# jamesmshihua/DiffusionPolicyOptimization

Measured on AMD Instinct MI355X. Metric: env-steps/sec + PPO-updates/sec, hopper-v2 64 envs 20 DDPM steps, 1/2/4/8 GPU, higher is better.
Workload: dtype bf16; 1 GPU; hopper-medium-v2 DPPO fine-tune iteration: 64 envs/GPU x 500 chunks (Ta=4), K=20 DDPM steps (K'=10), 5 PPO epochs x minibatch 50000, bf16 denoiser, synthetic linear env; env=synthetic, global_envs=64, chunks_per_rollout=500, parallelism=single GPU, batch_semantics=global minibatch 50000 rows = the reference's (50000 per rank)

## Files before the change

### diffusionpolicyoptimization_amd/csrc/update.hip

```cpp
#include <stdlib.h>
#include <mutex>
#include <vector>
#include "dppo_ppo.h"

enum { EXTRA_NONE = 0, EXTRA_ONES = 1, EXTRA_ONEHOT = 2 };
#define DW_MAXP 8
#define DW_TN 128
#ifndef DPPO_DW_LINE
#define DPPO_DW_LINE 128
#endif
#define DW_LINE DPPO_DW_LINE
#define DW_CPL (DW_LINE / 16)
#define DW_FPI (64 / DW_CPL)
#define DW_BOPB (DW_TN * DW_LINE)
static_assert(DW_LINE == 64 || DW_LINE == 128, "DPPO_DW_LINE must be 64 or 128");

template <int WK, int RC = 8> struct DWGeom {
    static constexpr int W = WK / 32;
    static constexpr int AOPB = WK * DW_LINE;
    static constexpr int SLOT = AOPB + DW_BOPB + 1024;
    static constexpr int RING0 = 160 * 1024 / SLOT < 8 ? 160 * 1024 / SLOT : 8;
    static constexpr int RING = RING0 < RC ? RING0 : RC;
    static constexpr int AI = WK / DW_FPI / W;
    static constexpr int BI = DW_TN / DW_FPI / W;
    static_assert(RING * SLOT <= 160 * 1024, "dW ring exceeds the CU's LDS");
};

struct DWProb {
    const void* XT; const void* DT; float* G; float* Gx;
    int Kx, N, extra, ktiles, ntiles;
};
struct DWArgs {
    DWProb p[DW_MAXP];
    int tile_start[DW_MAXP + 1];
    int nprob, nchunks, mchunk;
    float out_scale;
    size_t ldm;
    const int8_t* seg;
    const int* rows_dev;
};

typedef __attribute__((address_space(3))) void lds_void_t;

template <class P>
__device__ inline u32x4 extra_frag(int extra, int q, const int8_t* seg_lds) {
    using AT = typename P::AT;
    AT e[P::EPL];
    if (extra == EXTRA_ONES) {
#pragma unroll
        for (int i = 0; i < P::EPL; ++i) e[i] = P::cvt(1.f);
    } else {
        const uint64_t w = P::EPL == 8 ? *reinterpret_cast<const uint64_t*>(seg_lds)
                                       : (uint64_t)*reinterpret_cast<const uint32_t*>(seg_lds);
#pragma unroll
        for (int i = 0; i < P::EPL; ++i) e[i] = P::cvt((int)(int8_t)(w >> (8 * i)) == q ? 1.f : 0.f);
    }
    return __builtin_bit_cast(u32x4, e);
}

__device__ inline int dw_swz(int f, int c) {
    if constexpr (DW_LINE == 128) return c ^ (f & 7);
    else return c ^ ((0x78 >> (2 * ((f >> 2) & 3))) & 3);
}
__device__ inline u32x4 dw_lds_frag(const uint8_t* img, int f, int c) {
    return *reinterpret_cast<const u32x4*>(img + f * DW_LINE + (dw_swz(f, c) << 4));
}

template <int N>
__device__ inline void vm_wait() {
    static_assert(N >= 0 && N < 64, "vmcnt is 6 bits");
    __builtin_amdgcn_s_waitcnt((N & 15) | ((N >> 4) << 14) | (7 << 4) | (15 << 8));
}

template <class P, int WK, int RC, bool EXTRA, bool SEGLD>
__device__ __forceinline__ void dw_loop(uint8_t* smem, const DWArgs& a, const DWProb& pr, int nst, size_t m_begin,
                                        int wave, int lane, const typename P::AT* const (&srcA)[DWGeom<WK, RC>::AI],
                                        const typename P::AT* const (&srcB)[DWGeom<WK, RC>::BI],
                                        f32x4 (&acc)[4][4], f32x4 (&acce)[4]) {
    using G = DWGeom<WK, RC>;
    constexpr int BK = DW_LINE / (int)sizeof(typename P::AT);
    constexpr int OPS = G::AI + G::BI + (SEGLD ? 1 : 0);
    const int wr = wave >> 1, wc = wave & 1;
    const int fr = lane & 15, cq = lane >> 4;
    auto issue = [&](int st) {
        uint8_t* base = smem + (st % G::RING) * G::SLOT;
        const size_t off = (size_t)st * BK;
#pragma unroll
        for (int i = 0; i < G::AI; ++i)
            __builtin_amdgcn_global_load_lds((void*)(srcA[i] + off), (lds_void_t*)(base + (wave + G::W * i) * 1024), 16,
                                             0, 0);
#pragma unroll
        for (int i = 0; i < G::BI; ++i)
            __builtin_amdgcn_global_load_lds((void*)(srcB[i] + off),
                                             (lds_void_t*)(base + G::AOPB + (wave + G::W * i) * 1024), 16, 0, 0);
        if constexpr (SEGLD) {
            const int8_t* sg = a.seg + m_begin + off + 4 * (lane < BK / 4 ? lane : 0);
            __builtin_amdgcn_global_load_lds((void*)sg, (lds_void_t*)(base + G::AOPB + DW_BOPB), 4, 0, 0);
        }
    };
#pragma unroll
    for (int p = 0; p < G::RING - 1; ++p)
        if (p < nst) issue(p);
    for (int st = 0; st < nst; ++st) {
        const int ahead = nst - 1 - st;
        if (ahead >= G::RING - 2) vm_wait<(G::RING - 2) * OPS>();
        else if (ahead == 1) vm_wait<OPS>();
        else vm_wait<0>();
        __builtin_amdgcn_s_barrier();
        asm volatile("" ::: "memory");
        if (st + G::RING - 1 < nst) issue(st + G::RING - 1);
        const uint8_t* imA = smem + (st % G::RING) * G::SLOT;
        const uint8_t* imB = imA + G::AOPB;
        const int8_t* seg_lds = (const int8_t*)(imB + DW_BOPB);
#pragma unroll
        for (int ks = 0; ks < DW_LINE / 64; ++ks) {
            u32x4 A[4], B[4];
#pragma unroll
            for (int i = 0; i < 4; ++i) {
                A[i] = dw_lds_frag(imA, wr * 64 + i * 16 + fr, ks * 4 + cq);
                B[i] = dw_lds_frag(imB, wc * 64 + i * 16 + fr, ks * 4 + cq);
            }
#pragma unroll
            for (int i = 0; i < 4; ++i)
#pragma unroll
                for (int j = 0; j < 4; ++j) acc[i][j] = P::mma(A[i], B[j], acc[i][j]);
            if constexpr (EXTRA) {
                const u32x4 AE = extra_frag<P>(pr.extra, fr, seg_lds + ks * P::KG + cq * P::EPL);
#pragma unroll
                for (int j = 0; j < 4; ++j) acce[j] = P::mma(AE, B[j], acce[j]);
            }
        }
    }
}

static int dw_device_cus() {
    static int n = [] {
        int dev = 0, c = 0;
        if (hipGetDevice(&dev) != hipSuccess || hipDeviceGetAttribute(&c, hipDeviceAttributeMultiprocessorCount, dev) != hipSuccess)
            c = 256;
        return c > 0 ? c : 256;
    }();
    return n;
}

template <class P, int WK, int RC>
__global__ __launch_bounds__(WK / 32 * 64) void dw_kernel(DWArgs a) {
    using AT = typename P::AT;
    using G = DWGeom<WK, RC>;
    constexpr int BK = DW_LINE / (int)sizeof(AT);
    constexpr int EPC = 16 / (int)sizeof(AT);
    __shared__ __attribute__((aligned(1024))) uint8_t smem[G::RING * G::SLOT];
    const int tid = threadIdx.x, lane = tid & 63, wave = tid >> 6;
    const int tiles_all = a.tile_start[a.nprob];
    const int total = tiles_all * a.nchunks;
    const int per = (total + 7) >> 3;
    const int lg = (int)(blockIdx.x & 7) * per + (int)(blockIdx.x >> 3);
    if (lg >= total) return;
    const int chunk = lg / tiles_all;
    const int tile = lg % tiles_all;
    int pi = 0;
    while (pi + 1 < a.nprob && tile >= a.tile_start[pi + 1]) ++pi;
    const DWProb& pr = a.p[pi];
    const int lt = tile - a.tile_start[pi];
    const int kt = lt / pr.ntiles, nt = lt % pr.ntiles;
    const int k_base = kt * WK, n_base = nt * DW_TN;
    const int wr = wave >> 1, wc = wave & 1;
    size_t lim = a.ldm, mchunk = (size_t)a.mchunk;
    if (a.rows_dev) {
        const size_t d64 = (size_t)(__builtin_amdgcn_readfirstlane(*a.rows_dev) + 63) / 64 * 64;
        lim = d64 < lim ? d64 : lim;
        mchunk = (lim + (size_t)a.nchunks * 64 - 1) / ((size_t)a.nchunks * 64) * 64;
    }
    const size_t m_begin = (size_t)chunk * mchunk;
    const size_t m_end = m_begin + mchunk < lim ? m_begin + mchunk : lim;
    if (m_begin >= m_end) return;
    const int nst = (int)((m_end - m_begin) / BK);
    const AT* XT = (const AT*)pr.XT;
    const AT* DT = (const AT*)pr.DT;
    const bool wg_extra = pr.extra != EXTRA_NONE && kt == 0;
    const bool do_extra = wg_extra && wr == 0;
    const bool seg_ld = do_extra && pr.extra == EXTRA_ONEHOT;

    const AT* srcA[G::AI];
    const AT* srcB[G::BI];
#pragma unroll
    for (int i = 0; i < G::AI; ++i) {
        const int f = (wave + G::W * i) * DW_FPI + lane / DW_CPL;
        const int c = dw_swz(f, lane % DW_CPL);
        int fa = k_base + f; fa = fa < pr.Kx ? fa : pr.Kx - 1;
        srcA[i] = XT + (size_t)fa * a.ldm + m_begin + c * EPC;
    }
#pragma unroll
    for (int i = 0; i < G::BI; ++i) {
        const int f = (wave + G::W * i) * DW_FPI + lane / DW_CPL;
        const int c = dw_swz(f, lane % DW_CPL);
        int fb = n_base + f; fb = fb < pr.N ? fb : pr.N - 1;
        srcB[i] = DT + (size_t)fb * a.ldm + m_begin + c * EPC;
    }
    f32x4 acc[4][4], acce[4];
#pragma unroll
    for (int i = 0; i < 4; ++i) {
        zero_acc(acce[i]);
#pragma unroll
        for (int j = 0; j < 4; ++j) zero_acc(acc[i][j]);
    }
    if (seg_ld) dw_loop<P, WK, RC, true, true>(smem, a, pr, nst, m_begin, wave, lane, srcA, srcB, acc, acce);
    else if (do_extra) dw_loop<P, WK, RC, true, false>(smem, a, pr, nst, m_begin, wave, lane, srcA, srcB, acc, acce);
    else dw_loop<P, WK, RC, false, false>(smem, a, pr, nst, m_begin, wave, lane, srcA, srcB, acc, acce);
#pragma unroll
    for (int i = 0; i < 4; ++i)
#pragma unroll
        for (int j = 0; j < 4; ++j) {
            const int n = n_base + wc * 64 + j * 16 + ccol(lane);
#pragma unroll
            for (int r = 0; r < 4; ++r) {
                const int k = k_base + wr * 64 + i * 16 + crow(lane, r);
                if (k < pr.Kx && n < pr.N) atomicAdd(pr.G + (size_t)k * pr.N + n, acc[i][j][r] * a.out_scale);
            }
        }
    if (do_extra) {
#pragma unroll
        for (int j = 0; j < 4; ++j) {
            const int n = n_base + wc * 64 + j * 16 + ccol(lane);
            if (n >= pr.N) continue;
#pragma unroll
            for (int r = 0; r < 4; ++r) {
                const int q = crow(lane, r);
                if (pr.extra == EXTRA_ONES) {
                    if (q == 0) atomicAdd(pr.Gx + n, acce[j][r] * a.out_scale);
                } else {
                    atomicAdd(pr.Gx + (size_t)q * pr.N + n, acce[j][r] * a.out_scale);
                }
            }
        }
    }
}

#ifndef TB_THREADS
#define TB_THREADS 1024
#endif
struct L2Back {
    const float* pl2;
    const float* gob;
    const uint8_t* wimg;
    float* gw;
    float* gb;
    int H, N, prec;
    uint32_t* zcnt;
    const int* zlist;
    const int* zn;
};
__device__ inline float packed_elem(const uint8_t* img, int K, int k, int n, int prec) {
    const bool two = prec == DPPO_BF16 || prec == DPPO_F16;
    const int KG = two ? 32 : 16, EPL = two ? 8 : 4;
    const int lane = (n & 15) + 16 * ((k % KG) / EPL);
    const size_t slot = ((size_t)(n >> 4) * packed_ksteps(K, KG) + k / KG) * 64 + lane;
    const uint8_t* e = img + slot * 16 + (size_t)(k % EPL) * (two ? 2 : 4);
    if (prec == DPPO_BF16) return (float)*(const __bf16*)e;
    if (prec == DPPO_F16) return (float)*(const _Float16*)e;
    return *(const float*)e;
}
template <int PREC>
__device__ inline float packed_elem_t(const uint8_t* img, int K, int k, int n) {
    constexpr bool two = PREC == DPPO_BF16 || PREC == DPPO_F16;
    constexpr int KG = two ? 32 : 16, EPL = two ? 8 : 4;
    const int lane = (n & 15) + 16 * ((k % KG) / EPL);
    const size_t slot = ((size_t)(n >> 4) * packed_ksteps(K, KG) + k / KG) * 64 + lane;
    const uint8_t* e = img + slot * 16 + (size_t)(k % EPL) * (two ? 2 : 4);
    if constexpr (PREC == DPPO_BF16) return (float)*(const __bf16*)e;
    else if constexpr (PREC == DPPO_F16) return (float)*(const _Float16*)e;
    else return *(const float*)e;
}
constexpr int L2B_ROWS = 4;
constexpr int L2B_MAXN = 32;
template <int PREC, int NJ, int NQ>
__device__ inline void l2_back_cols(const L2Back& a, int b, int t, int nt) {
    const int H = a.H, N = NQ < L2B_MAXN ? NQ : a.N;
    const int h0 = L2B_ROWS * b;
    float pv[L2B_ROWS + 1][NQ];
#pragma unroll
    for (int r = 0; r < L2B_ROWS; ++r)
#pragma unroll
        for (int q = 0; q < NQ; ++q) pv[r][q] = q < N ? a.pl2[(size_t)(h0 + r) * N + q] : 0.f;
#pragma unroll
    for (int q = 0; q < NQ; ++q) pv[L2B_ROWS][q] = q < N ? a.gob[q] : 0.f;
    constexpr int NW = NQ <= 16 ? NJ : 1;
    float w[NW][NQ];
    auto load_w = [&](int c, float* dst) {
// ... 1064 lines not shown

extern "C" int dppo_feistel_permute(int64_t first, int64_t count, int64_t n, uint64_t seed, int epoch, int64_t* out,
                                    void* stream) {
    DPPO_CHECK(n > 0 && count >= 0 && first >= 0, "dppo_feistel_permute: bad range");
    if (count == 0) return DPPO_OK;
    DPPO_CHECK(out, "dppo_feistel_permute: null out");
    const FeistelKey fk = feistel_key((uint64_t)n, seed, epoch);
    hipLaunchKernelGGL(feistel_kernel, dim3((unsigned)((count + 255) / 256)), dim3(256), 0, (hipStream_t)stream,
                       first, count, fk, out);
    DPPO_HIP(hipGetLastError());
    return DPPO_OK;
}

extern "C" int dppo_ppo_adv_stats(const float* advantages, int64_t total, int K_ft, uint64_t perm_seed, int epoch,
                                  int64_t start, int rows, const int64_t* row_index, double* adv_stats, void* stream) {
    DPPO_CHECK(advantages && adv_stats && total > 0 && K_ft > 0 && rows >= 0, "dppo_ppo_adv_stats: bad args");
    hipStream_t s = (hipStream_t)stream;
    DPPO_HIP(hipMemsetAsync(adv_stats, 0, 3 * sizeof(double), s));
    if (rows == 0) return DPPO_OK;
    const FeistelKey fk = feistel_key((uint64_t)total, perm_seed, epoch);
    const int blocks = dppo_cdiv(rows, 256) < 512 ? dppo_cdiv(rows, 256) : 512;
    hipLaunchKernelGGL(adv_stats_kernel, dim3(blocks), dim3(256), 0, s, advantages, fk, K_ft, start, rows, row_index,
                       adv_stats);
    DPPO_HIP(hipGetLastError());
    return DPPO_OK;
}

extern "C" int dppo_ppo_adv_stats_all(const float* advantages, int64_t total, int K_ft, uint64_t perm_seed, int epoch0,
                                      int n_epochs, int64_t rows_full, int n_batch, double* adv_stats, void* stream) {
    DPPO_CHECK(advantages && adv_stats && total > 0 && K_ft > 0 && rows_full > 0 && n_batch > 0 && n_epochs > 0,
               "dppo_ppo_adv_stats_all: bad args");
    DPPO_CHECK(n_epochs <= ADV_MAXE, "dppo_ppo_adv_stats_all: at most %d epochs", ADV_MAXE);
    DPPO_CHECK((uint64_t)total < ((uint64_t)1 << 32), "dppo_ppo_adv_stats_all: total exceeds 2^32");
    hipStream_t s = (hipStream_t)stream;
    const int nm = n_epochs * n_batch;
    DPPO_HIP(hipMemsetAsync(adv_stats, 0, (size_t)3 * nm * sizeof(double), s));
    AdvStatsAll a = {};
    for (int e = 0; e < n_epochs; ++e) a.fk[e] = feistel_key((uint64_t)total, perm_seed, epoch0 + e);
    a.nbatch = n_batch; a.KF = K_ft; a.rows_full = rows_full; a.total = total;
    const int64_t bx = dppo_cdiv((int)(rows_full < total ? rows_full : total), 256);
    const int blocks = bx < 64 ? (int)bx : 64;
    DppoKtScope kt(KT_ADV_STATS, s);
    hipLaunchKernelGGL(adv_stats_all_kernel, dim3(blocks, nm), dim3(256), 0, s, advantages, a, adv_stats);
    DPPO_HIP(hipGetLastError());
    return DPPO_OK;
}

extern "C" size_t dppo_ppo_workspace_bytes(const dppo_dims* d, int precision, int batch_rows) {
    Dims D;
    if (dppo_check_dims(d, &D) || batch_rows < 0) return 0;
    return make_ppo_workspace(D, precision, batch_rows, nullptr).total;
}

template <class P>
static int launch_dw(const DWArgs& a, int wk, hipStream_t s) {
    const int tiles = a.tile_start[a.nprob];
    const int64_t blocks = 8 * (((int64_t)tiles * a.nchunks + 7) / 8);
    if (wk == 256)
        hipLaunchKernelGGL((dw_kernel<P, 256, 8>), dim3((unsigned)blocks), dim3(DWGeom<256>::W * 64), 0, s, a);
    else if (wk == 128)
        hipLaunchKernelGGL((dw_kernel<P, 128, 8>), dim3((unsigned)blocks), dim3(DWGeom<128>::W * 64), 0, s, a);
    else
        hipLaunchKernelGGL((dw_kernel<P, 128, 3>), dim3((unsigned)blocks), dim3(128 / 32 * 64), 0, s, a);
    DPPO_HIP(hipGetLastError());
    return DPPO_OK;
}

constexpr int DW_TK = 256;

struct SideStream { hipStream_t stream; hipEvent_t fork, join; };
static SideStream* side_stream() {
    constexpr int MAXDEV = 16;
    thread_local SideStream ss[MAXDEV] = {};
    thread_local bool tried[MAXDEV] = {};
    int dev = 0;
    if (hipGetDevice(&dev) != hipSuccess || dev < 0 || dev >= MAXDEV) return nullptr;
    SideStream& e = ss[dev];
    if (!tried[dev]) {
        tried[dev] = true;
        if (hipStreamCreateWithFlags(&e.stream, hipStreamNonBlocking) != hipSuccess ||
            hipEventCreateWithFlags(&e.fork, hipEventDisableTiming) != hipSuccess ||
            hipEventCreateWithFlags(&e.join, hipEventDisableTiming) != hipSuccess) {
            (void)hipGetLastError();
            e.stream = nullptr;
        }
    }
    return e.stream ? &e : nullptr;
}


static int launch_time_bwd(const Dims& D, int precision, const float* gseg, const float* pl2, const float* pa0,
                           const void* packed_actor, const float* actor_params, float* ga, int nb, int TS, hipStream_t s,
                           bool l2_back = true) {
    const FlatOffsets FA = make_flat_offsets(D.IN, D.H, D.XD, D.TD);
    const MlpLayout L = make_mlp_layout(D.IN, D.H, D.XD, D.TD, precision, D.K);
    L2Back l2b = {pl2, ga + FA.out_b, (const uint8_t*)packed_actor + L.off[SEG_W_OUT], ga + FA.l2_w, ga + FA.l2_b, D.H,
                  D.XD, precision, nullptr, nullptr, nullptr};
    DPPO_CHECK(D.XD <= L2B_MAXN, "l2_back: action horizon x dim %d > %d", D.XD, L2B_MAXN);
    DPPO_CHECK(D.IN <= 256 && D.H % 4 == 0, "out_back: in_dim %d > 256", D.IN);
    int stage_g = 0;
    const size_t tsm0 = time_bwd_lds(D, nb, &stage_g);
    const size_t tsm = tsm0 > sizeof(float) * OB_RED * (TB_THREADS / 256) ? tsm0 : sizeof(float) * OB_RED * (TB_THREADS / 256);
    DPPO_CHECK(tsm <= 160 * 1024, "time_bwd: LDS staging %zu B exceeds 160 KB", tsm);
    const int per = TB_THREADS / 256;
    const int l2g = l2_back ? dppo_cdiv(D.H, L2B_ROWS) : 0, obg = dppo_cdiv(D.H, ob_rows(l2_nq(D.XD)));
    const int nq = l2_nq(D.XD);
    const void* fn = time_l2_bwd_fn(precision, nq);
    { const int rc_ = dppo_func_lds(fn, tsm); if (rc_) return rc_; }
    DppoKtScope kt(KT_TIME_BWD, s);
    const OutBack ob = make_out_back(D, precision, actor_params, pl2, pa0, ga);
    const dim3 grid(1 + dppo_cdiv(l2g > obg ? l2g : obg, per));
    int XD = D.XD, TD = D.TD, H = D.H;
    FlatOffsets fa = FA;
    const float* prm = actor_params;
    void* args[] = {(void*)&gseg, (void*)&prm, (void*)&ga, (void*)&fa, (void*)&XD, (void*)&TD, (void*)&H, (void*)&nb,
                    (void*)&TS, (void*)&stage_g, (void*)&l2b, (void*)&l2g, (void*)&ob, (void*)&obg};
    DPPO_HIP(hipLaunchKernel(fn, grid, dim3(TB_THREADS), args, tsm, s));
    DPPO_HIP(hipGetLastError());
    return DPPO_OK;
}

// ... 70 lines not shown
    const PpoWorkspace ws = make_ppo_workspace(D, precision, rows, (uint8_t*)workspace);
    DPPO_CHECK(ws.total < ((size_t)1 << 31), "dppo_ppo_minibatch: workspace for %d rows exceeds 2 GiB", rows);
    const FlatOffsets FA = make_flat_offsets(D.IN, D.H, D.XD, D.TD);
    const FlatOffsets FC = make_flat_offsets(D.SD, D.HC, 1, 0);
    float* ga = grads;
    float* gc = grads + FA.count;
    DPPO_CHECK(parts >= 1 && parts <= 5, "dppo_ppo_minibatch: bad part %d", parts);
    DPPO_CHECK(parts == 3 || adv_stats || parts == 2 || parts == 5,
               "dppo_ppo_minibatch_part: the actor half needs adv_stats");
    DPPO_CHECK((hp->flags & ~(DPPO_PPO_L2_DEFERRED | DPPO_PPO_LEARN_ETA | DPPO_PPO_PRECLEARED)) == 0,
               "dppo_ppo_minibatch: unknown flags 0x%x", hp->flags);
    const ZeroArgs z = minibatch_zero_args(D, ws, grads, metrics, parts);
    if (parts != 5 && !(hp->flags & DPPO_PPO_PRECLEARED)) {
        DppoKtScope kt(KT_ZERO, s);
        hipLaunchKernelGGL(zero_kernel, dim3(16), dim3(256), 0, s, z);
        DPPO_HIP(hipGetLastError());
    }
    DPPO_CHECK((uint64_t)total < ((uint64_t)1 << 32), "dppo_ppo_minibatch: %lld samples x steps exceed 2^32",
               (long long)total);
    const FeistelKey fk = feistel_key((uint64_t)total, perm_seed, epoch);
    const double* stats = adv_stats;
    if (!stats && parts != 2 && parts != 5) {
        const int blocks = dppo_cdiv(rows, 256) < 512 ? dppo_cdiv(rows, 256) : 512;
        hipLaunchKernelGGL(adv_stats_kernel, dim3(blocks), dim3(256), 0, s, advantages, fk, D.KF, start, rows,
                           row_index, ws.stats);
        DPPO_HIP(hipGetLastError());
        stats = ws.stats;
    }
    LossHP lh;
    lh.gamma_denoising = hp->gamma_denoising; lh.clip_coef = hp->clip_ploss_coef;
    lh.clip_coef_base = hp->clip_ploss_coef_base; lh.clip_coef_rate = hp->clip_ploss_coef_rate;
    lh.min_lp_std = hp->min_logprob_std; lh.vf_coef = hp->vf_coef; lh.norm_adv = hp->norm_adv;
    lh.reward_horizon = hp->reward_horizon;
    const float gscale = dppo_grad_scale_rows(precision, hp->global_rows);
    lh.grad_scale = hp->loss_scale / (float)hp->global_rows * gscale;
    lh.eta_unscale = (hp->flags & DPPO_PPO_LEARN_ETA) ? 1.f / gscale : 0.f;
    lh.clip_vloss = hp->clip_vloss_coef > 0.f && hp->old_values ? hp->clip_vloss_coef : 0.f;
    lh.old_values = lh.clip_vloss > 0.f ? hp->old_values : nullptr;
    const bool l2_def = (hp->flags & DPPO_PPO_L2_DEFERRED) != 0;

    ActorArgs aa = {};
    aa.packed = (const uint8_t*)packed_ft;
    aa.L = make_mlp_layout(D.IN, D.H, D.XD, D.TD, precision, D.K);
    aa.sched = sched; aa.obs = obs; aa.chains = chains;
    aa.XD = D.XD; aa.SD = D.SD; aa.TD = D.TD; aa.IN = D.IN; aa.H = D.H; aa.KF = D.KF; aa.Da = D.Da; aa.TS = D.TS;
    aa.mode = ROWS_TRAIN; aa.nrows = rows; aa.fk = fk; aa.start = start; aa.row_index = row_index;
    aa.lp_old = lp_old_mean; aa.adv = advantages; aa.adv_stats = stats; aa.hp = lh; aa.ws = ws; aa.metrics = metrics;

    CriticArgs ca = {};
    ca.packed = (const uint8_t*)packed_critic;
    ca.L = make_mlp_layout(D.SD, D.HC, 1, 0, precision);
    ca.obs = obs; ca.SD = D.SD; ca.HC = D.HC; ca.KF = D.KF; ca.mode = ROWS_TRAIN; ca.nrows = rows;
    ca.fk = fk; ca.start = start; ca.row_index = row_index; ca.returns = returns; ca.hp = lh; ca.ws = ws; ca.metrics = metrics;
    const int tk = DW_TK;
    const int* crit_rows_dev = nullptr;
    auto launch_grads = [&](bool actor, hipStream_t st) -> int {
        DWArgs w = {};
        int all_tiles = 0;
        if (!actor) w.rows_dev = crit_rows_dev;
        const size_t span = ws.ldm;
        const int wk = actor ? tk : 0, tke = wk ? wk : 128;
        auto add = [&](const void* XT, int Kx, const void* DT, int N, float* G, int extra, float* Gx) {
            all_tiles += dppo_cdiv(Kx, tke) * dppo_cdiv(N, DW_TN);
            DWProb& p = w.p[w.nprob];
            p.XT = XT; p.DT = DT; p.G = G; p.Gx = Gx; p.Kx = Kx; p.N = N; p.extra = extra;
            p.ktiles = dppo_cdiv(Kx, tke); p.ntiles = dppo_cdiv(N, DW_TN);
            w.tile_start[w.nprob + 1] = w.tile_start[w.nprob] + p.ktiles * p.ntiles;
            w.nprob++;
        };
        if (actor) {
            add(ws.a0T, D.IN, ws.dh1T, D.H, ga + FA.in_w, EXTRA_ONEHOT, ws.gseg);
            add(ws.u1T, D.H, ws.dh2T, D.H, ga + FA.l1_w, EXTRA_ONES, ga + FA.l1_b);
            add(ws.u2T, D.H, ws.dyT, D.XD, l2_def ? ga + FA.l2_w : ws.pl2, EXTRA_NONE, nullptr);
            add(ws.a0T, D.IN, ws.dyT, D.XD, ws.pa0, EXTRA_ONES, ga + FA.out_b);
        } else {
            add(ws.csT, D.SD, ws.cdh1T, D.HC, gc + FC.in_w, EXTRA_ONES, gc + FC.in_b);
            add(ws.cu1T, D.HC, ws.cdh2T, D.HC, gc + FC.l1_w, EXTRA_ONES, gc + FC.l1_b);
            add(ws.cu2T, D.HC, ws.cdvT, 1, ws.cpl2, EXTRA_NONE, nullptr);
            add(ws.ch3T, D.HC, ws.cdvT, 1, gc + FC.out_w, EXTRA_ONES, gc + FC.out_b);
        }
        w.ldm = ws.ldm;
        w.seg = ws.seg;
        w.out_scale = 1.f / gscale;
        const int tiles = all_tiles;
        int nch = dw_device_cus() / tiles;
        if (nch > (int)(span / 768)) nch = (int)(span / 768);
        const int max_ch = (int)(span / 64);
        if (nch > max_ch) nch = max_ch;
        if (nch < 1) nch = 1;
        w.mchunk = (int)(dppo_cdiv((int)span, nch * 64) * 64);
        w.nchunks = dppo_cdiv((int)span, w.mchunk);
        DppoKtScope kt(actor ? KT_DW_ACTOR : KT_DW_CRITIC, st);
        return precision == DPPO_BF16 ? launch_dw<PolicyBF16>(w, wk, st)
             : precision == DPPO_F16  ? launch_dw<PolicyF16>(w, wk, st) : launch_dw<PolicyF32>(w, wk, st);
    };

    uint32_t* crit_cnt = nullptr;
    auto critic_rows = [&](hipStream_t st) -> int {
        if (!crit_dedup()) return DPPO_OK;
        const int64_t nsamp = total / D.KF;
        { const int rc_ = crit_count_scratch(nsamp, st, &crit_cnt); if (rc_) return rc_; }
        const int blocks = dppo_cdiv(rows, 256) < 512 ? dppo_cdiv(rows, 256) : 512;
        DppoKtScope kt(KT_CRIT_ROWS, st);
        hipLaunchKernelGGL(crit_rows_kernel, dim3(blocks), dim3(256), 0, st, row_index, start, rows, fk, D.KF, crit_cnt,
                           ws.crow_n, ws.crow_cnt);
        DPPO_HIP(hipGetLastError());
        ca.crow_n = ws.crow_n; ca.crow_mult = crit_cnt; ca.crow_cnt = ws.crow_cnt;
        crit_rows_dev = ws.crow_cnt;
        return DPPO_OK;
    };
    auto critic_tail = [&](hipStream_t st) {
        return launch_critic_l2_back(D, precision, ws.cpl2, packed_critic, gc, crit_cnt, ws.crow_n, ws.crow_cnt, st);
    };

    const float* pl2_src = l2_def ? ga + FA.l2_w : ws.pl2;
    auto actor_grads = [&]() -> int { return launch_grads(true, s); };
    auto actor_tail = [&]() -> int {
        return launch_time_bwd(D, precision, ws.gseg, pl2_src, ws.pa0, packed_ft, actor_params, ga, D.KF, D.TS, s,
                               !l2_def);
    };

    if (parts == 2) {
        rc = critic_rows(s);
        if (rc) return rc;
        rc = launch_critic_rowtile(ca, precision, s);
        if (rc) return rc;
        rc = launch_grads(false, s);
        if (rc) return rc;
        return critic_tail(s);
    }
    if (parts == 1 || parts == 4 || parts == 5) {
        if (parts != 5) {
            rc = launch_actor_rowtile(aa, precision, s);
            if (rc) return rc;
        }
        if (parts == 4) return DPPO_OK;
        rc = actor_grads();
        if (rc) return rc;
        return actor_tail();
    }
    SideStream* side = side_stream();
    if (side) {
        DPPO_HIP(hipEventRecord(side->fork, s));
        DPPO_HIP(hipStreamWaitEvent(side->stream, side->fork, 0));
        rc = critic_rows(side->stream);
        if (rc) return rc;
        rc = launch_critic_rowtile(ca, precision, side->stream);
// ... 76 lines not shown
__global__ __launch_bounds__(256) void seg_reduce_kernel(const AT* __restrict__ dT, const int8_t* __restrict__ seg,
                                                         size_t ldm, int nb, float* __restrict__ G, int H, float scale) {
    __shared__ float bins[4][64];
    const int n = blockIdx.x, tid = threadIdx.x, wave = tid >> 6;
    for (int i = tid; i < 4 * 64; i += 256) (&bins[0][0])[i] = 0.f;
    __syncthreads();
    const AT* row = dT + (size_t)n * ldm;
#pragma unroll 4
    for (size_t r = tid; r < ldm; r += 256) {
        const int q = seg[r];
        if (q >= 0 && q < nb) atomicAdd(&bins[wave][q], (float)row[r]);
    }
    __syncthreads();
    if (tid < nb) G[(size_t)tid * H + n] = ((bins[0][tid] + bins[1][tid]) + (bins[2][tid] + bins[3][tid])) * scale;
}

extern "C" int dppo_pretrain_minibatch(const dppo_dims* d, int precision, const void* packed_actor, const float* actor_params,
                                       const float* sched, const float* qsched, const float* x_start, const float* cond,
                                       const int32_t* t, const float* noise, int rows, int64_t global_rows,
                                       float loss_scale, void* workspace, float* grads, double* metrics, void* stream) {
    Dims D;
    int rc = dppo_check_dims(d, &D);
    if (rc) return rc;
    DPPO_CHECK(dppo_prec_ok(precision), "bad precision %d", precision);
    DPPO_CHECK(packed_actor && actor_params && sched && qsched && x_start && cond && t && noise && workspace && grads &&
               metrics, "dppo_pretrain_minibatch: null pointer");
    DPPO_CHECK(rows > 0 && global_rows >= rows, "dppo_pretrain_minibatch: bad rows / global_rows");
    DPPO_CHECK(D.TS == 1, "dppo_pretrain_minibatch: the time-embedding table must be unstrided (time_stride 1)");
    DPPO_CHECK(D.K <= 64, "dppo_pretrain_minibatch: denoising_steps > 64 unsupported (bucket sums)");
    hipStream_t s = (hipStream_t)stream;
    const PpoWorkspace ws = make_ppo_workspace(D, precision, rows, (uint8_t*)workspace);
    DPPO_CHECK(ws.total < ((size_t)1 << 31), "dppo_pretrain_minibatch: workspace for %d rows exceeds 2 GiB", rows);
    const FlatOffsets FA = make_flat_offsets(D.IN, D.H, D.XD, D.TD);
    float* ga = grads;
    ZeroArgs z = {};
    z.p[0] = grads; z.n[0] = FA.count * sizeof(float);
    z.p[1] = metrics; z.n[1] = 16 * sizeof(double);
    z.p[2] = ws.pl2; z.n[2] = (size_t)((const uint8_t*)ws.gseg - (const uint8_t*)ws.pl2);
    hipLaunchKernelGGL(zero_kernel, dim3(256), dim3(256), 0, s, z);
    DPPO_HIP(hipGetLastError());

    ActorArgs aa = {};
    aa.packed = (const uint8_t*)packed_actor;
    aa.L = make_mlp_layout(D.IN, D.H, D.XD, D.TD, precision, D.K);
    aa.sched = sched; aa.obs = cond; aa.chains = x_start;
    aa.XD = D.XD; aa.SD = D.SD; aa.TD = D.TD; aa.IN = D.IN; aa.H = D.H; aa.KF = D.K; aa.Da = D.Da; aa.TS = 1;
    aa.mode = ROWS_PRETRAIN; aa.nrows = rows; aa.ws = ws; aa.metrics = metrics;
    aa.tsteps = t; aa.noise = noise; aa.qsched = qsched;
    const float gscale = dppo_grad_scale_rows(precision, global_rows);
    aa.pre_scale = 2.f * loss_scale / ((float)global_rows * (float)D.XD) * gscale;
    rc = launch_actor_rowtile(aa, precision, s);
    if (rc) return rc;

    const int tk = DW_TK;
    DWArgs w = {};
    auto add = [&](const void* XT, int Kx, const void* DT, int N, float* G, int extra, float* Gx) {
        DWProb& p = w.p[w.nprob];
        p.XT = XT; p.DT = DT; p.G = G; p.Gx = Gx; p.Kx = Kx; p.N = N; p.extra = extra;
        p.ktiles = dppo_cdiv(Kx, tk); p.ntiles = dppo_cdiv(N, DW_TN);
        w.tile_start[w.nprob + 1] = w.tile_start[w.nprob] + p.ktiles * p.ntiles;
        w.nprob++;
    };
    add(ws.a0T, D.IN, ws.dh1T, D.H, ga + FA.in_w, EXTRA_NONE, nullptr);
    add(ws.u1T, D.H, ws.dh2T, D.H, ga + FA.l1_w, EXTRA_ONES, ga + FA.l1_b);
    add(ws.u2T, D.H, ws.dyT, D.XD, ws.pl2, EXTRA_NONE, nullptr);
    add(ws.a0T, D.IN, ws.dyT, D.XD, ws.pa0, EXTRA_ONES, ga + FA.out_b);
    w.ldm = ws.ldm;
    w.seg = ws.seg;
    w.out_scale = 1.f / gscale;
    const int tiles = w.tile_start[w.nprob];
    int nch = dw_device_cus() / tiles;
    const int max_ch = (int)(ws.ldm / 64);
    if (nch > max_ch) nch = max_ch;
    if (nch < 1) nch = 1;
    w.mchunk = (int)(dppo_cdiv((int)ws.ldm, nch * 64) * 64);
    w.nchunks = dppo_cdiv((int)ws.ldm, w.mchunk);
    rc = precision == DPPO_BF16 ? launch_dw<PolicyBF16>(w, tk, s)
       : precision == DPPO_F16  ? launch_dw<PolicyF16>(w, tk, s) : launch_dw<PolicyF32>(w, tk, s);
    if (rc) return rc;
    const float inv = 1.f / gscale;
    if (precision == DPPO_BF16)
        hipLaunchKernelGGL(seg_reduce_kernel<__bf16>, dim3(D.H), dim3(256), 0, s, (const __bf16*)ws.dh1T, ws.seg, ws.ldm,
                           D.K, ws.gseg, D.H, inv);
    else if (precision == DPPO_F16)
        hipLaunchKernelGGL(seg_reduce_kernel<_Float16>, dim3(D.H), dim3(256), 0, s, (const _Float16*)ws.dh1T, ws.seg,
                           ws.ldm, D.K, ws.gseg, D.H, inv);
    else
        hipLaunchKernelGGL(seg_reduce_kernel<float>, dim3(D.H), dim3(256), 0, s, (const float*)ws.dh1T, ws.seg, ws.ldm,
                           D.K, ws.gseg, D.H, inv);
    DPPO_HIP(hipGetLastError());
    return launch_time_bwd(D, precision, ws.gseg, ws.pl2, ws.pa0, packed_actor, actor_params, ga, D.K, 1, s);
}
```

Measured before the change: 3.920 million env-steps/s.

## Pick per-problem dW tile shapes and split rows by tile cost

The weight-gradient kernel now chooses a tile geometry for each sub-problem: wide, narrow-K or narrow-N, with separate wave counts and LDS budgets for the actor and critic networks. It also assigns each sub-problem its own row-chunk count in proportion to tile cost, instead of using one chunking for every problem. The aim is to stop wasting MFMA work and LDS traffic on thin layers such as the N=1 critic head and the small-K input layers, and to balance work across CUs. In exchange, the kernel carries more template instantiations and a runtime geometry branch, and the configurable DW_LINE option is removed.

```diff
diff --git a/diffusionpolicyoptimization_amd/csrc/update.hip b/diffusionpolicyoptimization_amd/csrc/update.hip
--- a/diffusionpolicyoptimization_amd/csrc/update.hip
+++ b/diffusionpolicyoptimization_amd/csrc/update.hip
@@ -5,35 +5,51 @@
 
 enum { EXTRA_NONE = 0, EXTRA_ONES = 1, EXTRA_ONEHOT = 2 };
 #define DW_MAXP 8
-#define DW_TN 128
-#ifndef DPPO_DW_LINE
-#define DPPO_DW_LINE 128
-#endif
-#define DW_LINE DPPO_DW_LINE
+#define DW_LINE 128
 #define DW_CPL (DW_LINE / 16)
 #define DW_FPI (64 / DW_CPL)
-#define DW_BOPB (DW_TN * DW_LINE)
-static_assert(DW_LINE == 64 || DW_LINE == 128, "DPPO_DW_LINE must be 64 or 128");
-
-template <int WK, int RC = 8> struct DWGeom {
-    static constexpr int W = WK / 32;
-    static constexpr int AOPB = WK * DW_LINE;
-    static constexpr int SLOT = AOPB + DW_BOPB + 1024;
-    static constexpr int RING0 = 160 * 1024 / SLOT < 8 ? 160 * 1024 / SLOT : 8;
-    static constexpr int RING = RING0 < RC ? RING0 : RC;
-    static constexpr int AI = WK / DW_FPI / W;
-    static constexpr int BI = DW_TN / DW_FPI / W;
-    static_assert(RING * SLOT <= 160 * 1024, "dW ring exceeds the CU's LDS");
+
+template <int W_, int TA_, int TB_, int WR_, int LDSB> struct DWGeom {
+    static constexpr int W = W_, TA = TA_, TB = TB_, WR = WR_, WC = W_ / WR_;
+    static constexpr int MI = TA / WR / 16, MJ = TB / WC / 16;
+    static constexpr int AOPB = TA * DW_LINE;
+    static constexpr int BOPB = TB * DW_LINE;
+    static constexpr int SLOT = AOPB + BOPB + 1024;
+    static constexpr int RING = LDSB / SLOT < 8 ? LDSB / SLOT : 8;
+    static constexpr int AI = TA / DW_FPI / W;
+    static constexpr int BI = TB / DW_FPI / W;
+    static_assert(WR * WC == W && MI * WR * 16 == TA && MJ * WC * 16 == TB, "dW tile does not split over its waves");
+    static_assert(AI * DW_FPI * W == TA && BI * DW_FPI * W == TB && AI > 0 && BI > 0, "dW stage copies are uneven");
+    static_assert(RING >= 3 && RING * SLOT <= 160 * 1024, "dW ring");
+};
+enum { DW_WIDE = 0, DW_NARK = 1, DW_NARN = 2, DW_NGEOM = 3 };
+template <int NET> struct DWNet;
+template <> struct DWNet<0> {
+    static constexpr int W = 8, LDSB = 160 * 1024;
+    using Wide = DWGeom<W, 256, 128, 4, LDSB>;
+    using NarK = DWGeom<W, 64, 256, 1, LDSB>;
+    using NarN = DWGeom<W, 256, 64, 8, LDSB>;
+};
+template <> struct DWNet<1> {
+    static constexpr int W = 4, LDSB = 3 * (2 * 128 * DW_LINE + 1024);
+    using Wide = DWGeom<W, 128, 128, 2, LDSB>;
+    using NarK = DWGeom<W, 64, 128, 1, LDSB>;
+    using NarN = DWGeom<W, 128, 32, 4, LDSB>;
+};
+template <class N_> struct DWNetInfo {
+    static constexpr int mx(int a, int b) { return a > b ? a : b; }
+    static constexpr int LDS = mx(N_::Wide::RING * N_::Wide::SLOT, mx(N_::NarK::RING * N_::NarK::SLOT, N_::NarN::RING * N_::NarN::SLOT));
 };
 
 struct DWProb {
     const void* XT; const void* DT; float* G; float* Gx;
-    int Kx, N, extra, ktiles, ntiles;
+    int Kx, N, extra, geom, ktiles, ntiles;
+    int nchunks, mchunk;
 };
 struct DWArgs {
     DWProb p[DW_MAXP];
-    int tile_start[DW_MAXP + 1];
-    int nprob, nchunks, mchunk;
+    int unit_start[DW_MAXP + 1];
+    int nprob;
     float out_scale;
     size_t ldm;
     const int8_t* seg;
@@ -58,10 +74,7 @@
     return __builtin_bit_cast(u32x4, e);
 }
 
-__device__ inline int dw_swz(int f, int c) {
-    if constexpr (DW_LINE == 128) return c ^ (f & 7);
-    else return c ^ ((0x78 >> (2 * ((f >> 2) & 3))) & 3);
-}
+__device__ inline int dw_swz(int f, int c) { return c ^ (f & 7); }
 __device__ inline u32x4 dw_lds_frag(const uint8_t* img, int f, int c) {
     return *reinterpret_cast<const u32x4*>(img + f * DW_LINE + (dw_swz(f, c) << 4));
 }
@@ -72,15 +85,14 @@
     __builtin_amdgcn_s_waitcnt((N & 15) | ((N >> 4) << 14) | (7 << 4) | (15 << 8));
 }
 
-template <class P, int WK, int RC, bool EXTRA, bool SEGLD>
+template <class P, class G, bool EXTRA, bool SEGLD>
 __device__ __forceinline__ void dw_loop(uint8_t* smem, const DWArgs& a, const DWProb& pr, int nst, size_t m_begin,
-                                        int wave, int lane, const typename P::AT* const (&srcA)[DWGeom<WK, RC>::AI],
-                                        const typename P::AT* const (&srcB)[DWGeom<WK, RC>::BI],
-                                        f32x4 (&acc)[4][4], f32x4 (&acce)[4]) {
-    using G = DWGeom<WK, RC>;
+                                        int wave, int lane, const typename P::AT* const (&srcA)[G::AI],
+                                        const typename P::AT* const (&srcB)[G::BI],
+                                        f32x4 (&acc)[G::MI][G::MJ], f32x4 (&acce)[G::MJ]) {
     constexpr int BK = DW_LINE / (int)sizeof(typename P::AT);
     constexpr int OPS = G::AI + G::BI + (SEGLD ? 1 : 0);
-    const int wr = wave >> 1, wc = wave & 1;
+    const int wr = wave / G::WC, wc = wave % G::WC;
     const int fr = lane & 15, cq = lane >> 4;
     auto issue = [&](int st) {
         uint8_t* base = smem + (st % G::RING) * G::SLOT;
@@ -95,7 +107,7 @@
                                              (lds_void_t*)(base + G::AOPB + (wave + G::W * i) * 1024), 16, 0, 0);
         if constexpr (SEGLD) {
             const int8_t* sg = a.seg + m_begin + off + 4 * (lane < BK / 4 ? lane : 0);
-            __builtin_amdgcn_global_load_lds((void*)sg, (lds_void_t*)(base + G::AOPB + DW_BOPB), 4, 0, 0);
+            __builtin_amdgcn_global_load_lds((void*)sg, (lds_void_t*)(base + G::AOPB + G::BOPB), 4, 0, 0);
         }
     };
 #pragma unroll
@@ -111,23 +123,22 @@
         if (st + G::RING - 1 < nst) issue(st + G::RING - 1);
         const uint8_t* imA = smem + (st % G::RING) * G::SLOT;
         const uint8_t* imB = imA + G::AOPB;
-        const int8_t* seg_lds = (const int8_t*)(imB + DW_BOPB);
+        const int8_t* seg_lds = (const int8_t*)(imB + G::BOPB);
 #pragma unroll
         for (int ks = 0; ks < DW_LINE / 64; ++ks) {
-            u32x4 A[4], B[4];
-#pragma unroll
-            for (int i = 0; i < 4; ++i) {
-                A[i] = dw_lds_frag(imA, wr * 64 + i * 16 + fr, ks * 4 + cq);
-                B[i] = dw_lds_frag(imB, wc * 64 + i * 16 + fr, ks * 4 + cq);
-            }
-#pragma unroll
-            for (int i = 0; i < 4; ++i)
-#pragma unroll
-                for (int j = 0; j < 4; ++j) acc[i][j] = P::mma(A[i], B[j], acc[i][j]);
+            u32x4 A[G::MI], B[G::MJ];
+#pragma unroll
+            for (int i = 0; i < G::MI; ++i) A[i] = dw_lds_frag(imA, (wr * G::MI + i) * 16 + fr, ks * 4 + cq);
+#pragma unroll
+            for (int j = 0; j < G::MJ; ++j) B[j] = dw_lds_frag(imB, (wc * G::MJ + j) * 16 + fr, ks * 4 + cq);
+#pragma unroll
+            for (int i = 0; i < G::MI; ++i)
+#pragma unroll
+                for (int j = 0; j < G::MJ; ++j) acc[i][j] = P::mma(A[i], B[j], acc[i][j]);
             if constexpr (EXTRA) {
                 const u32x4 AE = extra_frag<P>(pr.extra, fr, seg_lds + ks * P::KG + cq * P::EPL);
 #pragma unroll
-                for (int j = 0; j < 4; ++j) acce[j] = P::mma(AE, B[j], acce[j]);
+                for (int j = 0; j < G::MJ; ++j) acce[j] = P::mma(AE, B[j], acce[j]);
             }
         }
     }
@@ -143,38 +154,14 @@
     return n;
 }
 
-template <class P, int WK, int RC>
-__global__ __launch_bounds__(WK / 32 * 64) void dw_kernel(DWArgs a) {
+template <class P, class G>
+__device__ __forceinline__ void dw_tile(uint8_t* smem, const DWArgs& a, const DWProb& pr, int kt, int nt,
+                                        size_t m_begin, int nst) {
     using AT = typename P::AT;
-    using G = DWGeom<WK, RC>;
-    constexpr int BK = DW_LINE / (int)sizeof(AT);
     constexpr int EPC = 16 / (int)sizeof(AT);
-    __shared__ __attribute__((aligned(1024))) uint8_t smem[G::RING * G::SLOT];
     const int tid = threadIdx.x, lane = tid & 63, wave = tid >> 6;
-    const int tiles_all = a.tile_start[a.nprob];
-    const int total = tiles_all * a.nchunks;
-    const int per = (total + 7) >> 3;
-    const int lg = (int)(blockIdx.x & 7) * per + (int)(blockIdx.x >> 3);
-    if (lg >= total) return;
-    const int chunk = lg / tiles_all;
-    const int tile = lg % tiles_all;
-    int pi = 0;
-    while (pi + 1 < a.nprob && tile >= a.tile_start[pi + 1]) ++pi;
-    const DWProb& pr = a.p[pi];
-    const int lt = tile - a.tile_start[pi];
-    const int kt = lt / pr.ntiles, nt = lt % pr.ntiles;
-    const int k_base = kt * WK, n_base = nt * DW_TN;
-    const int wr = wave >> 1, wc = wave & 1;
-    size_t lim = a.ldm, mchunk = (size_t)a.mchunk;
-    if (a.rows_dev) {
-        const size_t d64 = (size_t)(__builtin_amdgcn_readfirstlane(*a.rows_dev) + 63) / 64 * 64;
-        lim = d64 < lim ? d64 : lim;
-        mchunk = (lim + (size_t)a.nchunks * 64 - 1) / ((size_t)a.nchunks * 64) * 64;
-    }
-    const size_t m_begin = (size_t)chunk * mchunk;
-    const size_t m_end = m_begin + mchunk < lim ? m_begin + mchunk : lim;
-    if (m_begin >= m_end) return;
-    const int nst = (int)((m_end - m_begin) / BK);
+    const int k_base = kt * G::TA, n_base = nt * G::TB;
+    const int wr = wave / G::WC, wc = wave % G::WC;
     const AT* XT = (const AT*)pr.XT;
     const AT* DT = (const AT*)pr.DT;
     const bool wg_extra = pr.extra != EXTRA_NONE && kt == 0;
@@ -197,31 +184,31 @@
         int fb = n_base + f; fb = fb < pr.N ? fb : pr.N - 1;
         srcB[i] = DT + (size_t)fb * a.ldm + m_begin + c * EPC;
     }
-    f32x4 acc[4][4], acce[4];
-#pragma unroll
-    for (int i = 0; i < 4; ++i) {
-        zero_acc(acce[i]);
-#pragma unroll
-        for (int j = 0; j < 4; ++j) zero_acc(acc[i][j]);
-    }
-    if (seg_ld) dw_loop<P, WK, RC, true, true>(smem, a, pr, nst, m_begin, wave, lane, srcA, srcB, acc, acce);
-    else if (do_extra) dw_loop<P, WK, RC, true, false>(smem, a, pr, nst, m_begin, wave, lane, srcA, srcB, acc, acce);
-    else dw_loop<P, WK, RC, false, false>(smem, a, pr, nst, m_begin, wave, lane, srcA, srcB, acc, acce);
-#pragma unroll
-    for (int i = 0; i < 4; ++i)
-#pragma unroll
-        for (int j = 0; j < 4; ++j) {
-            const int n = n_base + wc * 64 + j * 16 + ccol(lane);
+    f32x4 acc[G::MI][G::MJ], acce[G::MJ];
+#pragma unroll
+    for (int j = 0; j < G::MJ; ++j) {
+        zero_acc(acce[j]);
+#pragma unroll
+        for (int i = 0; i < G::MI; ++i) zero_acc(acc[i][j]);
+    }
+    if (seg_ld) dw_loop<P, G, true, true>(smem, a, pr, nst, m_begin, wave, lane, srcA, srcB, acc, acce);
+    else if (do_extra) dw_loop<P, G, true, false>(smem, a, pr, nst, m_begin, wave, lane, srcA, srcB, acc, acce);
+    else dw_loop<P, G, false, false>(smem, a, pr, nst, m_begin, wave, lane, srcA, srcB, acc, acce);
+#pragma unroll
+    for (int i = 0; i < G::MI; ++i)
+#pragma unroll
+        for (int j = 0; j < G::MJ; ++j) {
+            const int n = n_base + (wc * G::MJ + j) * 16 + ccol(lane);
 #pragma unroll
             for (int r = 0; r < 4; ++r) {
-                const int k = k_base + wr * 64 + i * 16 + crow(lane, r);
+                const int k = k_base + (wr * G::MI + i) * 16 + crow(lane, r);
                 if (k < pr.Kx && n < pr.N) atomicAdd(pr.G + (size_t)k * pr.N + n, acc[i][j][r] * a.out_scale);
             }
         }
     if (do_extra) {
 #pragma unroll
-        for (int j = 0; j < 4; ++j) {
-            const int n = n_base + wc * 64 + j * 16 + ccol(lane);
+        for (int j = 0; j < G::MJ; ++j) {
+            const int n = n_base + (wc * G::MJ + j) * 16 + ccol(lane);
             if (n >= pr.N) continue;
 #pragma unroll
             for (int r = 0; r < 4; ++r) {
@@ -234,6 +221,37 @@
             }
         }
     }
+}
+
+template <class P, int NET>
+__global__ __launch_bounds__(DWNet<NET>::W * 64) void dw_kernel(DWArgs a) {
+    using AT = typename P::AT;
+    using NT = DWNet<NET>;
+    constexpr int BK = DW_LINE / (int)sizeof(AT);
+    __shared__ __attribute__((aligned(1024))) uint8_t smem[DWNetInfo<NT>::LDS];
+    const int total = a.unit_start[a.nprob];
+    const int per = (total + 7) >> 3;
+    const int lg = (int)(blockIdx.x & 7) * per + (int)(blockIdx.x >> 3);
+    if (lg >= total) return;
+    int pi = 0;
+    while (pi + 1 < a.nprob && lg >= a.unit_start[pi + 1]) ++pi;
+    const DWProb& pr = a.p[pi];
+    const int unit = lg - a.unit_start[pi], tiles = pr.ktiles * pr.ntiles;
+    const int chunk = unit / tiles, lt = unit % tiles;
+    const int kt = lt / pr.ntiles, nt = lt % pr.ntiles;
+    size_t lim = a.ldm, mchunk = (size_t)pr.mchunk;
+    if (a.rows_dev) {
+        const size_t d64 = (size_t)(__builtin_amdgcn_readfirstlane(*a.rows_dev) + 63) / 64 * 64;
+        lim = d64 < lim ? d64 : lim;
+        mchunk = (lim + (size_t)pr.nchunks * 64 - 1) / ((size_t)pr.nchunks * 64) * 64;
+    }
+    const size_t m_begin = (size_t)chunk * mchunk;
+    const size_t m_end = m_begin + mchunk < lim ? m_begin + mchunk : lim;
+    if (m_begin >= m_end) return;
+    const int nst = (int)((m_end - m_begin) / BK);
+    if (pr.geom == DW_WIDE) dw_tile<P, typename NT::Wide>(smem, a, pr, kt, nt, m_begin, nst);
+    else if (pr.geom == DW_NARK) dw_tile<P, typename NT::NarK>(smem, a, pr, kt, nt, m_begin, nst);
+    else dw_tile<P, typename NT::NarN>(smem, a, pr, kt, nt, m_begin, nst);
 }
 
 #ifndef TB_THREADS
@@ -1404,21 +1422,51 @@
     return make_ppo_workspace(D, precision, batch_rows, nullptr).total;
 }
 
+static void dw_tile_edges(int net, int geom, int* ta, int* tb) {
+    auto set = [&](auto g) { *ta = decltype(g)::TA; *tb = decltype(g)::TB; };
+    if (net == 0) { if (geom == DW_WIDE) set(DWNet<0>::Wide{}); else if (geom == DW_NARK) set(DWNet<0>::NarK{}); else set(DWNet<0>::NarN{}); }
+    else          { if (geom == DW_WIDE) set(DWNet<1>::Wide{}); else if (geom == DW_NARK) set(DWNet<1>::NarK{}); else set(DWNet<1>::NarN{}); }
+}
+static void dw_add(DWArgs& w, int net, const void* XT, int Kx, const void* DT, int N, float* G, int extra, float* Gx) {
+    DWProb& p = w.p[w.nprob++];
+    p.XT = XT; p.DT = DT; p.G = G; p.Gx = Gx; p.Kx = Kx; p.N = N; p.extra = extra;
+    int ta, tb;
+    dw_tile_edges(net, DW_NARN, &ta, &tb);
+    const int narn_tb = tb;
+    dw_tile_edges(net, DW_NARK, &ta, &tb);
+    p.geom = N <= narn_tb ? DW_NARN : Kx <= ta ? DW_NARK : DW_WIDE;
+    dw_tile_edges(net, p.geom, &ta, &tb);
+    p.ktiles = dppo_cdiv(Kx, ta); p.ntiles = dppo_cdiv(N, tb);
+}
+static void dw_plan(DWArgs& w, int net, size_t span, int min_rows) {
+    int64_t cost[DW_MAXP], all = 0;
+    for (int i = 0; i < w.nprob; ++i) {
+        int ta, tb;
+        dw_tile_edges(net, w.p[i].geom, &ta, &tb);
+        cost[i] = ta + tb;
+        all += cost[i] * w.p[i].ktiles * w.p[i].ntiles;
+    }
+    w.unit_start[0] = 0;
+    for (int i = 0; i < w.nprob; ++i) {
+        DWProb& p = w.p[i];
+        int nch = (int)((int64_t)dw_device_cus() * cost[i] / all);
+        if (nch > (int)(span / min_rows)) nch = (int)(span / min_rows);
+        if (nch < 1) nch = 1;
+        p.mchunk = (int)(dppo_cdiv((int)span, nch * 64) * 64);
+        p.nchunks = dppo_cdiv((int)span, p.mchunk);
+        w.unit_start[i + 1] = w.unit_start[i] + p.ktiles * p.ntiles * p.nchunks;
+    }
+}
 template <class P>
-static int launch_dw(const DWArgs& a, int wk, hipStream_t s) {
-    const int tiles = a.tile_start[a.nprob];
-    const int64_t blocks = 8 * (((int64_t)tiles * a.nchunks + 7) / 8);
-    if (wk == 256)
-        hipLaunchKernelGGL((dw_kernel<P, 256, 8>), dim3((unsigned)blocks), dim3(DWGeom<256>::W * 64), 0, s, a);
-    else if (wk == 128)
-        hipLaunchKernelGGL((dw_kernel<P, 128, 8>), dim3((unsigned)blocks), dim3(DWGeom<128>::W * 64), 0, s, a);
+static int launch_dw(const DWArgs& a, int net, hipStream_t s) {
+    const int64_t blocks = 8 * (((int64_t)a.unit_start[a.nprob] + 7) / 8);
+    if (net == 0)
+        hipLaunchKernelGGL((dw_kernel<P, 0>), dim3((unsigned)blocks), dim3(DWNet<0>::W * 64), 0, s, a);
     else
-        hipLaunchKernelGGL((dw_kernel<P, 128, 3>), dim3((unsigned)blocks), dim3(128 / 32 * 64), 0, s, a);
+        hipLaunchKernelGGL((dw_kernel<P, 1>), dim3((unsigned)blocks), dim3(DWNet<1>::W * 64), 0, s, a);
     DPPO_HIP(hipGetLastError());
     return DPPO_OK;
 }
-
-constexpr int DW_TK = 256;
 
 struct SideStream { hipStream_t stream; hipEvent_t fork, join; };
 static SideStream* side_stream() {
@@ -1595,47 +1643,29 @@
     ca.L = make_mlp_layout(D.SD, D.HC, 1, 0, precision);
     ca.obs = obs; ca.SD = D.SD; ca.HC = D.HC; ca.KF = D.KF; ca.mode = ROWS_TRAIN; ca.nrows = rows;
     ca.fk = fk; ca.start = start; ca.row_index = row_index; ca.returns = returns; ca.hp = lh; ca.ws = ws; ca.metrics = metrics;
-    const int tk = DW_TK;
     const int* crit_rows_dev = nullptr;
     auto launch_grads = [&](bool actor, hipStream_t st) -> int {
         DWArgs w = {};
-        int all_tiles = 0;
         if (!actor) w.rows_dev = crit_rows_dev;
-        const size_t span = ws.ldm;
-        const int wk = actor ? tk : 0, tke = wk ? wk : 128;
-        auto add = [&](const void* XT, int Kx, const void* DT, int N, float* G, int extra, float* Gx) {
-            all_tiles += dppo_cdiv(Kx, tke) * dppo_cdiv(N, DW_TN);
-            DWProb& p = w.p[w.nprob];
-            p.XT = XT; p.DT = DT; p.G = G; p.Gx = Gx; p.Kx = Kx; p.N = N; p.extra = extra;
-            p.ktiles = dppo_cdiv(Kx, tke); p.ntiles = dppo_cdiv(N, DW_TN);
-            w.tile_start[w.nprob + 1] = w.tile_start[w.nprob] + p.ktiles * p.ntiles;
-            w.nprob++;
-        };
+        const int net = actor ? 0 : 1;
         if (actor) {
-            add(ws.a0T, D.IN, ws.dh1T, D.H, ga + FA.in_w, EXTRA_ONEHOT, ws.gseg);
-            add(ws.u1T, D.H, ws.dh2T, D.H, ga + FA.l1_w, EXTRA_ONES, ga + FA.l1_b);
-            add(ws.u2T, D.H, ws.dyT, D.XD, l2_def ? ga + FA.l2_w : ws.pl2, EXTRA_NONE, nullptr);
-            add(ws.a0T, D.IN, ws.dyT, D.XD, ws.pa0, EXTRA_ONES, ga + FA.out_b);
+            dw_add(w, net, ws.a0T, D.IN, ws.dh1T, D.H, ga + FA.in_w, EXTRA_ONEHOT, ws.gseg);
+            dw_add(w, net, ws.u1T, D.H, ws.dh2T, D.H, ga + FA.l1_w, EXTRA_ONES, ga + FA.l1_b);
+            dw_add(w, net, ws.u2T, D.H, ws.dyT, D.XD, l2_def ? ga + FA.l2_w : ws.pl2, EXTRA_NONE, nullptr);
+            dw_add(w, net, ws.a0T, D.IN, ws.dyT, D.XD, ws.pa0, EXTRA_ONES, ga + FA.out_b);
         } else {
-            add(ws.csT, D.SD, ws.cdh1T, D.HC, gc + FC.in_w, EXTRA_ONES, gc + FC.in_b);
-            add(ws.cu1T, D.HC, ws.cdh2T, D.HC, gc + FC.l1_w, EXTRA_ONES, gc + FC.l1_b);
-            add(ws.cu2T, D.HC, ws.cdvT, 1, ws.cpl2, EXTRA_NONE, nullptr);
-            add(ws.ch3T, D.HC, ws.cdvT, 1, gc + FC.out_w, EXTRA_ONES, gc + FC.out_b);
+            dw_add(w, net, ws.csT, D.SD, ws.cdh1T, D.HC, gc + FC.in_w, EXTRA_ONES, gc + FC.in_b);
+            dw_add(w, net, ws.cu1T, D.HC, ws.cdh2T, D.HC, gc + FC.l1_w, EXTRA_ONES, gc + FC.l1_b);
+            dw_add(w, net, ws.cu2T, D.HC, ws.cdvT, 1, ws.cpl2, EXTRA_NONE, nullptr);
+            dw_add(w, net, ws.ch3T, D.HC, ws.cdvT, 1, gc + FC.out_w, EXTRA_ONES, gc + FC.out_b);
         }
         w.ldm = ws.ldm;
         w.seg = ws.seg;
         w.out_scale = 1.f / gscale;
-        const int tiles = all_tiles;
-        int nch = dw_device_cus() / tiles;
-        if (nch > (int)(span / 768)) nch = (int)(span / 768);
-        const int max_ch = (int)(span / 64);
-        if (nch > max_ch) nch = max_ch;
-        if (nch < 1) nch = 1;
-        w.mchunk = (int)(dppo_cdiv((int)span, nch * 64) * 64);
-        w.nchunks = dppo_cdiv((int)span, w.mchunk);
+        dw_plan(w, net, ws.ldm, 768);
         DppoKtScope kt(actor ? KT_DW_ACTOR : KT_DW_CRITIC, st);
-        return precision == DPPO_BF16 ? launch_dw<PolicyBF16>(w, wk, st)
-             : precision == DPPO_F16  ? launch_dw<PolicyF16>(w, wk, st) : launch_dw<PolicyF32>(w, wk, st);
+        return precision == DPPO_BF16 ? launch_dw<PolicyBF16>(w, net, st)
+             : precision == DPPO_F16  ? launch_dw<PolicyF16>(w, net, st) : launch_dw<PolicyF32>(w, net, st);
     };
 
     uint32_t* crit_cnt = nullptr;
@@ -1818,31 +1848,17 @@
     rc = launch_actor_rowtile(aa, precision, s);
     if (rc) return rc;
 
-    const int tk = DW_TK;
     DWArgs w = {};
-    auto add = [&](const void* XT, int Kx, const void* DT, int N, float* G, int extra, float* Gx) {
-        DWProb& p = w.p[w.nprob];
-        p.XT = XT; p.DT = DT; p.G = G; p.Gx = Gx; p.Kx = Kx; p.N = N; p.extra = extra;
-        p.ktiles = dppo_cdiv(Kx, tk); p.ntiles = dppo_cdiv(N, DW_TN);
-        w.tile_start[w.nprob + 1] = w.tile_start[w.nprob] + p.ktiles * p.ntiles;
-        w.nprob++;
-    };
-    add(ws.a0T, D.IN, ws.dh1T, D.H, ga + FA.in_w, EXTRA_NONE, nullptr);
-    add(ws.u1T, D.H, ws.dh2T, D.H, ga + FA.l1_w, EXTRA_ONES, ga + FA.l1_b);
-    add(ws.u2T, D.H, ws.dyT, D.XD, ws.pl2, EXTRA_NONE, nullptr);
-    add(ws.a0T, D.IN, ws.dyT, D.XD, ws.pa0, EXTRA_ONES, ga + FA.out_b);
+    dw_add(w, 0, ws.a0T, D.IN, ws.dh1T, D.H, ga + FA.in_w, EXTRA_NONE, nullptr);
+    dw_add(w, 0, ws.u1T, D.H, ws.dh2T, D.H, ga + FA.l1_w, EXTRA_ONES, ga + FA.l1_b);
+    dw_add(w, 0, ws.u2T, D.H, ws.dyT, D.XD, ws.pl2, EXTRA_NONE, nullptr);
+    dw_add(w, 0, ws.a0T, D.IN, ws.dyT, D.XD, ws.pa0, EXTRA_ONES, ga + FA.out_b);
     w.ldm = ws.ldm;
     w.seg = ws.seg;
     w.out_scale = 1.f / gscale;
-    const int tiles = w.tile_start[w.nprob];
-    int nch = dw_device_cus() / tiles;
-    const int max_ch = (int)(ws.ldm / 64);
-    if (nch > max_ch) nch = max_ch;
-    if (nch < 1) nch = 1;
-    w.mchunk = (int)(dppo_cdiv((int)ws.ldm, nch * 64) * 64);
-    w.nchunks = dppo_cdiv((int)ws.ldm, w.mchunk);
-    rc = precision == DPPO_BF16 ? launch_dw<PolicyBF16>(w, tk, s)
-       : precision == DPPO_F16  ? launch_dw<PolicyF16>(w, tk, s) : launch_dw<PolicyF32>(w, tk, s);
+    dw_plan(w, 0, ws.ldm, 64);
+    rc = precision == DPPO_BF16 ? launch_dw<PolicyBF16>(w, 0, s)
+       : precision == DPPO_F16  ? launch_dw<PolicyF16>(w, 0, s) : launch_dw<PolicyF32>(w, 0, s);
     if (rc) return rc;
     const float inv = 1.f / gscale;
     if (precision == DPPO_BF16)
```

After: 3.855 million env-steps/s. 1.7% lower.
